# ActiveVisionLab/NeFeS

Measured on AMD Instinct MI355X. Metric: rays/s (fwd+bwd) at 640x480x(64+128) samples, 8x256 MLP, higher is better.
Workload: dtype f32; 1 GPU; BASELINE configs[1]: 7-Scenes-stairs geometry, 64+128 samples, 8x256 MLP + 16-ch feature head; 640x480, random seed-0 weights, fwd + bwd to the 3x4 pose; parallelism=rows/1

## Files before the change

__graft_entry__.py:

```python
import os
import subprocess
import sys

ROOT = os.path.dirname(os.path.abspath(__file__))
if ROOT not in sys.path:
    sys.path.insert(0, ROOT)


def build() -> None:
    env = dict(os.environ)
    env.setdefault("PYTORCH_ROCM_ARCH", "gfx950")
    jobs = str(min(6, os.cpu_count() or 1))
    subprocess.run(["make", "-C", os.path.join(ROOT, "nefes_amd", "csrc"), "-j", jobs], check=True, env=env)
    import py_compile
    for name in ("ref_cpu.py", "refine_cpu.py", "hashgrid_ref.py"):
        py_compile.compile(os.path.join(ROOT, "oracle", name), doraise=True)
    import nefes_amd
    from nefes_amd import lib
    assert lib.load().nefes_version() == lib.ABI_VERSION


def smoke() -> None:
    import torch
    from nefes_amd import lib
    from nefes_amd.field import NeRFH_NFF
    from nefes_amd.render import render
    from oracle import ref_cpu as O
    import types
# ... 43 lines not shown
```

nefes_amd/csrc/field_fwd_h3.hip:

```cpp
#include "field_h3_instances.h"
#ifdef NEFES_TU_W128
#define NEFES_SLAB_KIB 16
#else
#define NEFES_SLAB_KIB 32
#endif
#include <stdio.h>
#include <stdlib.h>
#if defined(NEFES_TU_W128) || !defined(H3_NO_ACC_READ_ASM)
#define NEFES_ASM_READS_ACC
#define NEFES_FENCE_TILES
#endif
#if defined(NEFES_TU_W128)
#define NEFES_ACC_VGPR_FORM
#endif

#ifndef NEFES_FWD_CONSUMER_BIAS
#define NEFES_FWD_CONSUMER_BIAS 1
#endif
#include "field_common.h"
#include "../../include/nefes_hip.h"

#include "field_x6.h"
#include "hashgrid.h"
#if !defined(NEFES_TU_W128) && !defined(H3_NO_ACC_READ_ASM)
#define H3_ACC_READ_ASM
#endif
#include "field_h3.h"
#define NEFES_H3_SLOTS 2

struct FieldFwdH3Args {
    const char* stream;
    const float* bias;
    uint32_t n_slabs, bias_floats, scale_off;
    const float* rays_o;
    const float* rays_d;
    const float* z;
    const float* pts;
    const float* xyz_enc;
    const float* viewdirs;
    float* raw_t;
    uint32_t* masks;
    int N, S, R, C;
    long long M;
    int n_tiles;
    uint32_t s_magic, s_shift;
    float* acts;
    int rows;
    int z_row;
    const float2* hg_table;
    HgGeom hg;
    int gout;
};

template <int NT, int T0, int NX>
__device__ __forceinline__ void train_save_h3(float* tile_base, uint32_t voff, int row0, const f32x16 (&X)[NX], float inv) {
    float* p = tile_base + (size_t)(row0 >> 5) * 4096 + voff;
#pragma unroll
    for (int t = 0; t < NT; ++t)
#pragma unroll
        for (int r = 0; r < 16; ++r) {
#ifndef NEFES_TRAIN_NO_STORES
            __builtin_nontemporal_store(X[T0 + t][r] * inv, &p[t * 4096 + nefes_rho(0, r) * 16]);
#endif
        }
}

template <int MODEF, int ENC, int W = 256, int NTR = 1, bool TRAIN = false, bool FH = false>
__global__ __launch_bounds__(256, W == 128 ? 2 : 1) void field_fwd_h3_kernel(FieldFwdH3Args a) {
    constexpr bool FOLD = MODEF == NEFES_FIELD_FULL_FOLD;
    constexpr int MODE = FOLD ? NEFES_FIELD_FULL : MODEF;
    static_assert(NEFES_SLAB_KIB == (W == 128 ? NEFES_H3_FWD_SLAB_KIB_128 : NEFES_H3_FWD_SLAB_KIB), "ring slab size != the packer's for this width");
    static_assert(!FOLD || (MODE != NEFES_FIELD_SIGMA && !TRAIN), "the fold serves the head products of frozen networks");
    constexpr int NTW = W / 32, NTH = W / 64;
    constexpr int ES = ENC != NEFES_XYZ_FREQ10 ? NEFES_X_STEPS : NEFES_E_STEPS;
    constexpr int MW = 8 * (W / 64) + 4 * (W / 128), WT = (NTW + 1) / 2, WH = (NTH + 1) / 2;
    constexpr int NSEG = MODE == NEFES_FIELD_SIGMA ? NEFES_H3F_SIG + 1
                         : (MODE == NEFES_FIELD_STATIC ? NEFES_H3F_N_STATIC : (FOLD ? NEFES_H3FF_N : NEFES_H3F_N));
    extern __shared__ __attribute__((aligned(16))) char smem[];
    char* ring_base = smem;
    float* bias_lds = (float*)(smem + NEFES_H3_SLOTS * NEFES_SLAB_BYTES);
    float* e_lds = bias_lds + ((a.bias_floats + 63) / 64) * 64 + (threadIdx.x >> 6) * (ES * 64) + (threadIdx.x & 63);
    const int lane = threadIdx.x & 63;
    const int wave = __builtin_amdgcn_readfirstlane(threadIdx.x >> 6);
    const int j = lane & 31, h = lane >> 5;
    for (uint32_t i = threadIdx.x; i < a.bias_floats; i += 256) bias_lds[i] = a.bias[i];
    HgGeom* hg_lds = (HgGeom*)(bias_lds + ((a.bias_floats + 63) / 64) * 64 + 4 * ES * 64);
    if constexpr (ENC == NEFES_XYZ_HASHGRID_FUSED) {
        if (threadIdx.x == 0) *hg_lds = a.hg;
    }
    StagedRing ring;
    ring.init(a.stream, a.n_slabs, ring_base, wave, lane);
    const char* ring_lane = ring_base + lane * 16;
    const char* bias_half = (const char*)bias_lds + 16 * h;
    const int* tab_i = (const int*)(bias_lds + a.scale_off);
    const float* tab_f = bias_lds + a.scale_off;
    auto wexp = [&](int seg) { return tab_i[nefes_h3_tab_exp(nefes_h3f_seg(FOLD, seg))]; };
    auto rowb = [&](int seg) { return tab_f[nefes_h3_tab_bound(nefes_h3f_seg(FOLD, seg))]; };
    auto bmax = [&](int blk) { return tab_f[nefes_h3_tab_bias(NSEG, nefes_h3f_bias(FOLD, blk))]; };
    ring.prime(ring_lane);
    constexpr int B_SIG = 8 * W, B_FINAL = B_SIG + 32, B_DIR = B_FINAL + (FOLD ? 0 : W), B_RGB = B_DIR + W / 2,
                  B_T0 = B_RGB + 32 * NTR, B_T1 = B_T0 + W / 2, B_T2 = B_T1 + W / 2, B_TH = B_T2 + W / 2;
#pragma unroll 1
    for (int tile = blockIdx.x; tile < a.n_tiles; tile += gridDim.x) {
        auto locate = [&](uint32_t& m, uint32_t& ray, uint32_t& smp) {
            const uint32_t m_raw = (uint32_t)tile * 128u + (uint32_t)(wave * 32 + j);
            const bool ok = m_raw < (uint32_t)a.M;
            m = ok ? m_raw : (uint32_t)a.M - 1u;
            ray = a.s_magic ? __umulhi(m, a.s_magic) >> a.s_shift : m;
            smp = m - ray * (uint32_t)a.S;
            return ok;
        };
        uint32_t m, ray, smp;
        locate(m, ray, smp);
        float in_o[3] = {0.f, 0.f, 0.f}, in_d[3] = {0.f, 0.f, 0.f}, in_z = 0.f;
// ... 52 lines not shown
            return a.raw_t + ((size_t)rr * a.R * a.S + ss);
        };
        auto bias_at = [&](int off_floats, int es) { return BiasInitScaled{bias_half + off_floats * 4, pow2i(es)}; };
        constexpr bool CB = !TRAIN && W == 256 && NEFES_FWD_CONSUMER_BIAS;
        float2 nbias;
        f32x16 A[NTW], B[NTW];
        uint32_t bits[WT];
        auto clear_bits = [&]() {
#pragma unroll
            for (int w = 0; w < WT; ++w) bits[w] = 0u;
        };
        constexpr bool CAP = MODE != NEFES_FIELD_SIGMA;
        auto tau_of = [&](float M, int ew) {
            const int t = pick_exp(M);
            return t < 100 - ew ? t : 100 - ew;
        };
        auto sigma_head = [&](const f32x16 (&X)[NTW], int es_x, int tau_x) {
            f32x16 sg[1];
            float mdummy = 0.f;
            const int es = tau_x + wexp(NEFES_H3F_SIG);
            if constexpr (CB) {
                const char* bp8 = bias_half + 7 * W * 4;
                nbias = ReluBiasSplitH<false, NTW, WT>::prime(bp8);
                mma_run_h3<1, W / 16, 0, true>(ring, ring_lane, ReluBiasSplitH<false, NTW, WT>{X, bits, pow2i(tau_x - es_x), mdummy, bp8, pow2i(es_x), nbias},
                                               bias_at(B_SIG, es), sg);
            } else
            mma_run_h3<1, W / 16, 0, true>(ring, ring_lane, ReluSplitH<false, NTW, WT>{X, bits, pow2i(tau_x - es_x), mdummy},
                                           bias_at(B_SIG, es), sg);
            float* col = raw_col();
            if (col && h == 0) {
// ... 20 lines not shown
            if constexpr (CB) {                                                                                                \
                const char* bps = bias_half + ((L1_) - 2) * W * 4;                           \
                nbias = ReluBiasSplitH<CAP, NTW, WT>::prime(bps);                                                              \
                mma_run_h3<NTW, W / 16, 0, true>(ring, ring_lane, ReluBiasSplitH<CAP, NTW, WT>{A, bits, pow2i(tau - es_a), mx, bps, pow2i(es_a), nbias}, \
                                                 ZeroInit{}, B);                                                               \
            } else                                                                                                             \
            mma_run_h3<NTW, W / 16, 0, true>(ring, ring_lane, ReluSplitH<CAP, NTW, WT>{A, bits, pow2i(tau - es_a), mx},        \
                                             bias_at(((L1_) - 1) * W, tau + ew), B);                                           \
            M = rb_ * (pair_max(mx) * pow2i(-es_a)) + bm_;                                                                     \
            es_b = tau + ew;                                                                                                   \
            save_trunk(L1_, B, es_b);                                                                                          \
        }                                                                                                                      \
        put_masks(bits, WT);
        constexpr bool END8 = MODE == NEFES_FIELD_SIGMA || FOLD;
        constexpr int NPAIRS = END8 ? 3 : 4;
#pragma unroll 1
        for (int p = 0; p < NPAIRS; ++p) {
            const int l1 = 2 + 2 * p, l2 = l1 + 1;
            const int seg1 = l1 <= 5 ? l1 - 1 : l1;
            const int seg2 = l2 <= 5 ? l2 - 1 : (l2 <= 8 ? l2 : NEFES_H3F_FINAL);
            NEFES_FWD_EVEN_LAYER(l1, seg1)
            clear_bits();
            {
                const int ew = wexp(seg2);
                const int tau = tau_of(p == 1 ? fmaxf(M, mE) : M, ew);
                if (p == 3) sigma_head(B, es_b, tau_of(M, wexp(NEFES_H3F_SIG)));
                const float rb_ = rowb(seg2), bm_ = bmax(l2 <= 8 ? l2 - 1 : NEFES_H3BB_FINAL);
                const float rbe_ = p == 1 ? rowb(NEFES_H3F_L5E) : 0.f;
                float mx = 0.f;
                if constexpr (CB) {
                    const char* bps = bias_half + (l1 - 1) * W * 4;
                    nbias = ReluBiasSplitH<CAP, NTW, WT>::prime(bps);
                    const ReluBiasSplitH<CAP, NTW, WT> src{B, bits, pow2i(tau - es_b), mx, bps, pow2i(es_b), nbias};
                    mma_run_h3<NTW, W / 16, 0, true>(ring, ring_lane, src, ZeroInit{}, A);
                } else
                mma_run_h3<NTW, W / 16, 0, true>(ring, ring_lane, ReluSplitH<CAP, NTW, WT>{B, bits, pow2i(tau - es_b), mx},
                                                 bias_at(l2 <= 8 ? (l2 - 1) * W : B_FINAL, tau + ew), A);
                if (p == 1) mma_run_h3<NTW, ES / 8, 0, false>(ring, ring_lane, LdsSplitH{e_lds, pow2i(tau)}, ZeroInit{}, A);
                M = rb_ * (pair_max(mx) * pow2i(-es_b)) + (p == 1 ? rbe_ * mE : 0.f) + bm_;
                es_a = tau + ew;
                save_trunk(l2, A, es_a);
            }
            put_masks(bits, WT);
        }
        if constexpr (END8) { NEFES_FWD_EVEN_LAYER(8, NEFES_H3F_L8) }
#undef NEFES_FWD_EVEN_LAYER
        if constexpr (MODE == NEFES_FIELD_SIGMA) sigma_head(B, es_b, tau_of(M, wexp(NEFES_H3F_SIG)));
        if constexpr (MODE != NEFES_FIELD_SIGMA) {
            constexpr bool FULL = MODE == NEFES_FIELD_FULL;
            constexpr int NDT = FULL ? 2 * NTH : NTH;
            float v[3];
            {
                uint32_t mm, rr, ss;
                locate(mm, rr, ss);
#pragma unroll
                for (int c = 0; c < 3; ++c) v[c] = a.viewdirs[(size_t)rr * 3 + c];
            }
            float Dv[16];
            {
                float d14[NEFES_D_STEPS];
                embed_slots<NEFES_N_FREQ_DIR>(d14, v, h);
#pragma unroll
// ... 4 lines not shown
#pragma unroll
                for (int s = 0; s < NEFES_D_STEPS; ++s) __builtin_nontemporal_store(Dv[s], &pd[2 * s * 16]);
            }
            f32x16 dt[NDT];
            uint32_t bits2[WH];
            auto clear2 = [&]() {
#pragma unroll
                for (int w = 0; w < WH; ++w) bits2[w] = 0u;
            };
            struct Bias2 {
                BiasInitScaled a, b;
                __device__ __forceinline__ f32x16 operator()(int t) const { return t < NTH ? a(t) : b(t - NTH); }
            };
            int es_dt;
            if constexpr (FOLD) {
                sigma_head(B, es_b, tau_of(M, wexp(NEFES_H3F_SIG)));
                const int ew = wexp(NEFES_H3F_DT_H);
                const float mD = pair_max(array_max(Dv));
                const int tau = tau_of(fmaxf(M, mD), ew);
                const float rbh_ = rowb(NEFES_H3F_DT_H), rbd_ = rowb(NEFES_H3F_DT_D);
                const float bm_ = fmaxf(bmax(NEFES_H3BB_DIR), bmax(NEFES_H3BB_T0));
                float mx = 0.f;
                es_dt = tau + ew;
                clear_bits();
                if constexpr (CB) {
                    const char* bp8 = bias_half + 7 * W * 4;
                    nbias = ReluBiasSplitH<CAP, NTW, WT>::prime(bp8);
                    const ReluBiasSplitH<CAP, NTW, WT> src8{B, bits, pow2i(tau - es_b), mx, bp8, pow2i(es_b), nbias};
                    mma_run_h3<NDT, W / 16, 0, true>(ring, ring_lane, src8, Bias2{bias_at(B_DIR, es_dt), bias_at(B_T0, es_dt)}, dt);
                } else {
                    const ReluSplitH<CAP, NTW, WT> src8{B, bits, pow2i(tau - es_b), mx};
                    mma_run_h3<NDT, W / 16, 0, true>(ring, ring_lane, src8, Bias2{bias_at(B_DIR, es_dt), bias_at(B_T0, es_dt)}, dt);
                }
                mma_run_h3<NDT, 2, 0, false>(ring, ring_lane, ArraySplitH<16>{Dv, pow2i(tau)}, ZeroInit{}, dt);
                M = rbh_ * (pair_max(mx) * pow2i(-es_b)) + rbd_ * mD + bm_;
                put_masks(bits, WT);
            } else {
                const int ew = wexp(NEFES_H3F_DT_H);
                const float mD = pair_max(array_max(Dv));
                const int tau = tau_of(fmaxf(M, mD), ew);
                float mx = 0.f;
                es_dt = tau + ew;
                if constexpr (CB) {
                    const char* bpf = bias_half + B_FINAL * 4;
                    nbias = ReluBiasSplitH<false, 1, 1>::prime(bpf);
                    const IdentBiasSplitH<NTW> srcf{A, pow2i(tau - es_a), mx, bpf, pow2i(es_a), nbias};
                    if constexpr (FULL) mma_run_h3<NDT, W / 16, 0, true>(ring, ring_lane, srcf, Bias2{bias_at(B_DIR, es_dt), bias_at(B_T0, es_dt)}, dt);
                    else mma_run_h3<NDT, W / 16, 0, true>(ring, ring_lane, srcf, bias_at(B_DIR, es_dt), dt);
// ... 109 lines not shown
    }
}

static void magic_div(uint32_t d, uint32_t& magic, uint32_t& shift) {
    if (d == 1) { magic = 0; shift = 0; return; }
    uint32_t l = 0;
    while ((1ull << l) < d) ++l;
    const uint64_t p = 31 + l;
    magic = (uint32_t)(((1ull << p) + d - 1) / d);
    shift = (uint32_t)(p - 32);
}

template <int MODE, int ENC, int W = 256, int NTR = 1, bool TRAIN = false, bool FH = false>
static int launch_h3(const FieldFwdH3Args& a, hipStream_t st) {
    constexpr int ES_ = ENC != NEFES_XYZ_FREQ10 ? NEFES_X_STEPS : NEFES_E_STEPS;
    const size_t lds = (size_t)NEFES_H3_SLOTS * NEFES_SLAB_BYTES + ((a.bias_floats + 63) / 64) * 256 + (size_t)4 * ES_ * 64 * 4
                       + (ENC == NEFES_XYZ_HASHGRID_FUSED ? 512 : 0);
    static_assert(sizeof(HgGeom) <= 512, "the level geometry's LDS slot");
    auto k = field_fwd_h3_kernel<MODE, ENC, W, NTR, TRAIN, FH>;
    hipError_t e = hipFuncSetAttribute((const void*)k, hipFuncAttributeMaxDynamicSharedMemorySize, (int)lds);
    if (e != hipSuccess) return (int)e;
    int dev = 0, cus = 256;
    (void)hipGetDevice(&dev);
    (void)hipDeviceGetAttribute(&cus, hipDeviceAttributeMultiprocessorCount, dev);
    const int per_cu = W == 128 ? 2 : 1;
    int grid = a.n_tiles < cus * per_cu ? a.n_tiles : cus * per_cu;
    if (const char* cap = getenv("NEFES_DEBUG_MAX_GRID")) {
        const int c = atoi(cap);
        if (c > 0 && c < grid) grid = c;
    }
    hipLaunchKernelGGL(k, dim3(grid), dim3(256), lds, st, a);
// ... 77 lines not shown
    int rc = nefes_blob_info(desc, &info);
    if (rc) return rc;
    *si = info.stream[k.mode == NEFES_FIELD_SIGMA ? NEFES_STREAM_FWD_SIGMA_H3
                      : (k.mode == NEFES_FIELD_STATIC ? NEFES_STREAM_FWD_STATIC_H3 : NEFES_STREAM_FWD_FULL_H3)];
    return si->n_slabs == 0 ? NEFES_E_UNSUPPORTED : 0;
}

static int h3_fwd_args(const NefesNetDesc* desc, const void* packed, const NefesH3FwdKey& k, int N, int S,
                       const NefesHashGridDesc* grid, FieldFwdH3Args& a) {
    NefesStreamInfo si;
    int rc = h3_fwd_stream(desc, k, &si);
    if (rc) return rc;
    a.stream = (const char*)packed + si.slab_off;
    a.bias = (const float*)((const char*)packed + si.bias_off);
    a.n_slabs = si.n_slabs; a.bias_floats = si.bias_floats; a.scale_off = si.scale_off;
    if (k.enc == NEFES_XYZ_HASHGRID_FUSED) {
        rc = hg_geometry(grid, &a.hg, nullptr);
        if (rc) return rc;
        if (a.hg.n_levels != 16) return NEFES_E_UNSUPPORTED;
    }
    a.gout = k.fh ? k.w / 2 : 0;
    a.N = N; a.S = S; a.C = k.fh ? a.gout + 1 : desc->feat_dim;
    a.R = k.mode == NEFES_FIELD_SIGMA ? 1 : 3 + a.C + (k.mode == NEFES_FIELD_STATIC ? 1 : 6);
    a.M = (long long)N * S;
    if (a.M >= (1ll << 31) - 256) return NEFES_E_UNSUPPORTED;
    a.n_tiles = (int)((a.M + 127) / 128);
    a.rows = k.train ? nefes_train_row(desc->width, desc->feat_dim, NEFES_TB_END) : 0;
    magic_div((uint32_t)S, a.s_magic, a.s_shift);
    return 0;
}
// ... 99 lines not shown
```

nefes_amd/csrc/field_h3.h:

```cpp
#pragma once
#ifndef NEFES_H3_WIDE_MIN
#define NEFES_H3_WIDE_MIN 8
#endif
#ifndef NEFES_H3_WIDE_MAX
#define NEFES_H3_WIDE_MAX 64
#endif

typedef _Float16 f16x8 __attribute__((ext_vector_type(8)));

struct Split2 {
    u32x4 h, l;
};
__device__ __forceinline__ f16x8 as_f16x8(u32x4 v) {
    f16x8 r;
    __builtin_memcpy(&r, &v, 16);
    return r;
}
__device__ __forceinline__ f16x8 as_f16x8(f32x4 v) {
    f16x8 r;
    __builtin_memcpy(&r, &v, 16);
    return r;
}

__device__ __forceinline__ float pow2i(int e) {
// ... 81 lines not shown
    o.l[p] = l;
}

struct PairRegs {
    float x0, x1;
};
__device__ __forceinline__ float acc_read(const float& x) {
#if defined(H3_ACC_READ_ASM)
    float v;
    asm volatile("v_accvgpr_read_b32 %0, %1" : "=v"(v) : "a"(x));
    return v;
#else
    return x;
#endif
}
template <bool CAPTURE, int NX, int NWORDS, int T0 = 0>
struct ReluSplitH {
    const f32x16 (&X)[NX];
    uint32_t (&bits)[NWORDS];
    float r;
    float& m;
    __device__ __forceinline__ void stage_a(PairRegs& s, int q, int p) const {
        s.x0 = acc_read(X[T0 + (q >> 1)][(q & 1) * 8 + 2 * p]);
        s.x1 = acc_read(X[T0 + (q >> 1)][(q & 1) * 8 + 2 * p + 1]);
        if (CAPTURE) {
            mask_shift_in(bits[(8 * q + 2 * p) >> 5], s.x0);
            mask_shift_in(bits[(8 * q + 2 * p + 1) >> 5], s.x1);
        }
    }
    __device__ __forceinline__ void stage_b(PairRegs& s) const {
        s.x0 = relu1<false>(s.x0);
        s.x1 = relu1<false>(s.x1);
        max3_acc(m, s.x0, s.x1);
    }
    template <bool NOP>
    __device__ __forceinline__ void stage_c(Split2& o, int p, const PairRegs& s) const { split_pair_h<NOP>(o, p, s.x0, s.x1, r); }
    __device__ __forceinline__ void stage_c1(Split2& o, int p, const PairRegs& s) const { split_pair_hi(o, p, s.x0, s.x1, r); }
    template <bool NOP>
    __device__ __forceinline__ void stage_c2(Split2& o, int p, const PairRegs& s) const { split_pair_lo<NOP>(o, p, s.x0, s.x1, r); }
};
template <bool CAPTURE, int NX, int NWORDS>
struct ReluBiasSplitH {
    const f32x16 (&X)[NX];
    uint32_t (&bits)[NWORDS];
    float r;
    float& m;
    const char* bp;
    float bs;
    float2& nb;
    static __device__ __forceinline__ int pair_off(int q, int p) {
        const int r0 = (q & 1) * 8 + 2 * p;
        return ((q >> 1) * 32 + 8 * (r0 >> 2) + (r0 & 3)) * 4;
    }
    static __device__ __forceinline__ float2 prime(const char* bp_) { return *(const float2*)(bp_ + pair_off(0, 0)); }
    __device__ __forceinline__ void stage_a(PairRegs& s, int q, int p) const {
        const float2 b = nb;
        const int qn = p == 3 ? q + 1 : q, pn = p == 3 ? 0 : p + 1;
        nb = *(const float2*)(bp + pair_off(qn, pn));
        s.x0 = __builtin_fmaf(b.x, bs, acc_read(X[q >> 1][(q & 1) * 8 + 2 * p]));
        s.x1 = __builtin_fmaf(b.y, bs, acc_read(X[q >> 1][(q & 1) * 8 + 2 * p + 1]));
        if (CAPTURE) {
            mask_shift_in(bits[(8 * q + 2 * p) >> 5], s.x0);
            mask_shift_in(bits[(8 * q + 2 * p + 1) >> 5], s.x1);
        }
    }
    __device__ __forceinline__ void stage_b(PairRegs& s) const {
        s.x0 = relu1<false>(s.x0);
        s.x1 = relu1<false>(s.x1);
// ... 112 lines not shown

struct BiasInitScaled {
    const char* p;
    float s;
    __device__ __forceinline__ f32x16 operator()(int t) const {
        f32x16 c;
#pragma unroll
        for (int q = 0; q < 4; ++q) {
            const f32x4 b = *(const f32x4*)(p + (t * 32 + 8 * q) * 4);
            c[4 * q + 0] = b[0] * s; c[4 * q + 1] = b[1] * s; c[4 * q + 2] = b[2] * s; c[4 * q + 3] = b[3] * s;
        }
        return c;
    }
};

struct StagedRing {
    const char* src;
    uint32_t n_slabs;
    uint32_t g_next;
    uint32_t c_slot;
    uint32_t cur_off;
    uint32_t my_off;
    char* my_lds;
    f32x4 pf;
    f32x4 stage[NEFES_SLAB_PIECES];

    __device__ __forceinline__ void load_piece(int q) {
        stage[q] = *(const f32x4*)(src + (size_t)g_next * NEFES_SLAB_BYTES + my_off + q * 1024);
    }
    __device__ __forceinline__ void init(const char* stream, uint32_t nslabs, char* ring_base, int wave, int lane) {
        src = stream; n_slabs = nslabs;
        my_off = (uint32_t)(wave * NEFES_SLAB_PIECES * 1024 + lane * 16);
        my_lds = ring_base + my_off;
        g_next = 0; c_slot = 0; cur_off = 0;
#pragma unroll
        for (int q = 0; q < NEFES_SLAB_PIECES; ++q) load_piece(q);
#pragma unroll
        for (int q = 0; q < NEFES_SLAB_PIECES; ++q) *(f32x4*)(my_lds + q * 1024) = stage[q];
        g_next = n_slabs > 1 ? 1 : 0;
#pragma unroll
        for (int q = 0; q < NEFES_SLAB_PIECES; ++q) load_piece(q);
        g_next = (g_next + 1 == n_slabs) ? 0 : g_next + 1;
    }
    __device__ __forceinline__ void store_piece(int q) {
        *(f32x4*)(my_lds + (c_slot ^ 1u) * NEFES_SLAB_BYTES + q * 1024) = stage[q];
    }
    __device__ __forceinline__ void fetch_piece(int q) {
        load_piece(q);
        if (q == NEFES_SLAB_PIECES - 1) g_next = (g_next + 1 == n_slabs) ? 0 : g_next + 1;
    }
    __device__ __forceinline__ void issue_piece(int q) {
        *(f32x4*)(my_lds + (c_slot ^ 1u) * NEFES_SLAB_BYTES + q * 1024) = stage[q];
        load_piece(q);
        if (q == NEFES_SLAB_PIECES - 1) g_next = (g_next + 1 == n_slabs) ? 0 : g_next + 1;
    }
    __device__ __forceinline__ uint32_t acquire() {
        asm volatile("s_waitcnt lgkmcnt(0)" ::: "memory");
        __builtin_amdgcn_s_barrier();
        c_slot ^= 1u;
        return c_slot * NEFES_SLAB_BYTES;
    }
    __device__ __forceinline__ void prime(const char* ring_lane) {
        asm volatile("s_waitcnt lgkmcnt(0)" ::: "memory");
        __builtin_amdgcn_s_barrier();
        cur_off = 0;
        pf = *(const f32x4*)(ring_lane);
    }
    __device__ __forceinline__ void drain() {}
};

__device__ __forceinline__ void mfma_h3_asm(f32x16& c, const f32x4& a, const u32x4& b) {
    asm volatile("v_mfma_f32_32x32x16_f16 %0, %1, %2, %0" : "+a"(c) : "v"(a), "v"(b));
}
__device__ __forceinline__ void mfma_h3_asm_v(f32x16& c, const f32x4& a, const u32x4& b) {
    asm volatile("v_mfma_f32_32x32x16_f16 %0, %1, %2, %0" : "+v"(c) : "v"(a), "v"(b));
}
__device__ __forceinline__ void mfma_h3_asm_c0(f32x16& c, const f32x4& a, const u32x4& b) {
    asm volatile("v_mfma_f32_32x32x16_f16 %0, %1, %2, 0" : "=a"(c) : "v"(a), "v"(b));
}
__device__ __forceinline__ void mfma_h3_asm_v_c0(f32x16& c, const f32x4& a, const u32x4& b) {
    asm volatile("v_mfma_f32_32x32x16_f16 %0, %1, %2, 0" : "=v"(c) : "v"(a), "v"(b));
}
template <class T> struct h3_is_zero_init { static constexpr bool value = false; };
template <> struct h3_is_zero_init<ZeroInit> { static constexpr bool value = true; };
// ... 8 lines not shown
    constexpr int NSLAB = (NU + UPS - 1) / UPS;
    Split2 B0, B1;
    auto BQ = [&](int k) -> Split2& { return (k & 1) ? B1 : B0; };
    asm volatile("s_nop 13" ::: "memory");
#ifdef H3_WIDE_ENTRY_FENCE
    __builtin_amdgcn_sched_barrier(0);
    asm volatile("s_nop 7\n\ts_nop 7\n\ts_nop 1" ::: "memory");
    __builtin_amdgcn_sched_barrier(0);
#endif
    {
        PairRegs s0;
#pragma unroll
        for (int pp = 0; pp < 4; ++pp) {
            src.stage_a(s0, 0, pp);
            src.stage_b(s0);
            if (pp == 3) src.template stage_c<true>(B0, pp, s0);
            else src.template stage_c<false>(B0, pp, s0);
        }
    }
    constexpr bool C0 = FIRST && h3_is_zero_init<InitFn>::value
        ;
    if (FIRST && !C0) acc[T0] = init(0);
    const char* p = ring_lane + ring.cur_off;
    f32x4 ha0 = ring.pf, la0 = *(const f32x4*)(p + 1024);
    f32x4 ha1 = *(const f32x4*)(p + 2048), la1 = *(const f32x4*)(p + 3072);
    f32x4 ha2, la2;
    auto HA = [&](int k) -> f32x4& { return k % 3 == 0 ? ha0 : (k % 3 == 1 ? ha1 : ha2); };
    auto LA = [&](int k) -> f32x4& { return k % 3 == 0 ? la0 : (k % 3 == 1 ? la1 : la2); };
    PairRegs ps[4];
#pragma unroll
// ... 25 lines not shown
                    }
                    if (vt) mfma_h3_asm_v(acc[T0 + t], l0, B.h);
                    else mfma_h3_asm(acc[T0 + t], l0, B.h);
                }
                __builtin_amdgcn_sched_barrier(0);
                if (host) src.stage_a(ps[pp], q + 1, pp);
                if (tail) src.template stage_c2<false>(Bn, pp, ps[pp]);
                if (!host && uu != acq_u) h2 = *(const f32x4*)(pn);
                __builtin_amdgcn_sched_barrier(0);
                asm volatile("" ::"v"(l0), "v"(B.h));
                if (vt) mfma_h3_asm_v(acc[T0 + t], h0, B.l);
                else mfma_h3_asm(acc[T0 + t], h0, B.l);
                __builtin_amdgcn_sched_barrier(0);
                if (host) src.stage_b(ps[pp]);
                if (host && uu != acq_u) h2 = *(const f32x4*)(pn);
                if (!host) {
#pragma unroll
                    for (int qq = 0; qq < NEFES_SLAB_PIECES; ++qq)
                        if (piece_unit(qq) == uu) ring.store_piece(qq);
                }
                if (FIRST && !C0 && q == 0 && t + 1 < NT) {
                    acc[T0 + t + 1] = init(t + 1);
                }
                __builtin_amdgcn_sched_barrier(0);
                asm volatile("" ::"v"(B.l));
                if (vt) mfma_h3_asm_v(acc[T0 + t], h0, B.h);
                else mfma_h3_asm(acc[T0 + t], h0, B.h);
                __builtin_amdgcn_sched_barrier(0);
                if (host) src.stage_c1(Bn, pp, ps[pp]);
                if (!host) {
// ... 28 lines not shown

template <int NT, int KS16, int T0, bool FIRST = true, class SrcFn, class InitFn, int NACC, class Ring>
__device__ __forceinline__ void mma_run_h3_small(Ring& ring, const char* ring_lane, const SrcFn& src, const InitFn& init,
                                           f32x16 (&acc)[NACC]) {
    static_assert(T0 + NT <= NACC, "accumulator array too small");
    constexpr int UPS = (NEFES_SLAB_FRAGS / 4) / 2;
    constexpr int NU = KS16 * NT;
    constexpr int NSLAB = (NU + UPS - 1) / UPS;
    Split2 B, Bn;
    {
        PairRegs s0;
#pragma unroll
        for (int pp = 0; pp < 4; ++pp) {
            src.stage_a(s0, 0, pp);
            src.stage_b(s0);
            if (pp == 3) src.template stage_c<true>(B, pp, s0);
            else src.template stage_c<false>(B, pp, s0);
        }
    }
    Bn = B;
    if (FIRST) acc[T0] = init(0);
    const char* p = ring_lane + ring.cur_off;
    f32x4 ah = ring.pf, al = *(const f32x4*)(p + 1024);
#pragma unroll
    for (int sl = 0; sl < NSLAB; ++sl) {
        const int nu = (NU - sl * UPS) < UPS ? (NU - sl * UPS) : UPS;
#pragma unroll
        for (int uu = 0; uu < UPS; ++uu) {
            if (uu < nu) {
                const int u = sl * UPS + uu, q = u / NT, t = u % NT;
// ... 25 lines not shown
                            ring.issue_piece(qq);
                            __builtin_amdgcn_sched_barrier(0);
                        }
                }
                c = __builtin_amdgcn_mfma_f32_32x32x16_f16(Ah, Bl, c, 0, 0, 0);
                c = __builtin_amdgcn_mfma_f32_32x32x16_f16(Ah, Bh, c, 0, 0, 0);
                acc[T0 + t] = c;
                if (q + 1 < KS16) {
                    constexpr int STRIDE = NT >= 8 ? 2 : 1;
#pragma unroll
                    for (int pp = 0; pp < 4; ++pp)
                        if (NT >= 4 ? (t == pp * STRIDE + STRIDE - 1) : (t == (pp * NT) / 4)) {
                            PairRegs s1;
                            src.stage_a(s1, q + 1, pp);
                            src.stage_b(s1);
                            if (pp == 3) src.template stage_c<true>(Bn, pp, s1);
                            else src.template stage_c<false>(Bn, pp, s1);
#pragma unroll
                            for (int i = 0; i < 2; ++i) {
                                __builtin_amdgcn_sched_group_barrier(0x008, 1, 0);
                                __builtin_amdgcn_sched_group_barrier(0x002, 4, 0);
                            }
                        }
                }
                ah = nh;
            }
        }
    }
    ring.pf = ah;
    mfma_results_fence_tiles<12, NT, T0>(acc);
// ... 9 lines not shown
```

Measured before the change: 738,700 rays/s.

## Compute sigma head as an FP32 dot product fused into the next layer's staging

Instead of running the sigma head as a separate MFMA pass over a streamed weight slab, the forward kernel preloads the sigma weights into LDS as FP32. It accumulates the dot product with the ReLU'd trunk activations while they are staged for the following layer's matmul, finishing with a cross-half permlane swap. The weight ring now skips the sigma slab. This removes one slab fetch and a small MFMA run per tile, at the cost of extra FMAs and LDS reads inside the staging loop, more register pressure, and a slightly different rounding path.

```diff
diff --git a/__graft_entry__.py b/__graft_entry__.py
--- a/__graft_entry__.py
+++ b/__graft_entry__.py
@@ -11,7 +11,7 @@
     env = dict(os.environ)
     env.setdefault("PYTORCH_ROCM_ARCH", "gfx950")
     jobs = str(min(6, os.cpu_count() or 1))
-    subprocess.run(["make", "-C", os.path.join(ROOT, "nefes_amd", "csrc"), "-j", jobs], check=True, env=env)
+    subprocess.run(["make", "-C", os.path.join(ROOT, "nefes_amd", "csrc"), "-j", jobs, "all", "nodot"], check=True, env=env)
     import py_compile
     for name in ("ref_cpu.py", "refine_cpu.py", "hashgrid_ref.py"):
         py_compile.compile(os.path.join(ROOT, "oracle", name), doraise=True)
diff --git a/nefes_amd/csrc/field_fwd_h3.hip b/nefes_amd/csrc/field_fwd_h3.hip
--- a/nefes_amd/csrc/field_fwd_h3.hip
+++ b/nefes_amd/csrc/field_fwd_h3.hip
@@ -17,6 +17,9 @@
 #ifndef NEFES_FWD_CONSUMER_BIAS
 #define NEFES_FWD_CONSUMER_BIAS 1
 #endif
+#ifndef NEFES_FWD_SIGMA_DOT
+#define NEFES_FWD_SIGMA_DOT 1
+#endif
 #include "field_common.h"
 #include "../../include/nefes_hip.h"
 
@@ -27,6 +30,8 @@
 #endif
 #include "field_h3.h"
 #define NEFES_H3_SLOTS 2
+
+constexpr bool h3_fwd_sigma_dot(bool train) { return NEFES_FWD_SIGMA_DOT && !train; }
 
 struct FieldFwdH3Args {
     const char* stream;
@@ -50,6 +55,7 @@
     const float2* hg_table;
     HgGeom hg;
     int gout;
+    uint32_t sig_slab;
 };
 
 template <int NT, int T0, int NX>
@@ -71,6 +77,10 @@
     constexpr int MODE = FOLD ? NEFES_FIELD_FULL : MODEF;
     static_assert(NEFES_SLAB_KIB == (W == 128 ? NEFES_H3_FWD_SLAB_KIB_128 : NEFES_H3_FWD_SLAB_KIB), "ring slab size != the packer's for this width");
     static_assert(!FOLD || (MODE != NEFES_FIELD_SIGMA && !TRAIN), "the fold serves the head products of frozen networks");
+    constexpr bool DOT = h3_fwd_sigma_dot(TRAIN);
+    static_assert(!DOT || (W / 16) * 2048 == NEFES_SLAB_BYTES, "static_sigma's segment is not one slab of this stream");
+    static_assert(!DOT || !TRAIN, "TRAIN instances keep static_sigma's own run");
+    constexpr int WSIG_BYTES = DOT ? W * 4 : 0;
     constexpr int NTW = W / 32, NTH = W / 64;
     constexpr int ES = ENC != NEFES_XYZ_FREQ10 ? NEFES_X_STEPS : NEFES_E_STEPS;
     constexpr int MW = 8 * (W / 64) + 4 * (W / 128), WT = (NTW + 1) / 2, WH = (NTH + 1) / 2;
@@ -78,7 +88,8 @@
                          : (MODE == NEFES_FIELD_STATIC ? NEFES_H3F_N_STATIC : (FOLD ? NEFES_H3FF_N : NEFES_H3F_N));
     extern __shared__ __attribute__((aligned(16))) char smem[];
     char* ring_base = smem;
-    float* bias_lds = (float*)(smem + NEFES_H3_SLOTS * NEFES_SLAB_BYTES);
+    float* wsig_lds = (float*)(smem + NEFES_H3_SLOTS * NEFES_SLAB_BYTES);
+    float* bias_lds = (float*)(smem + NEFES_H3_SLOTS * NEFES_SLAB_BYTES + WSIG_BYTES);
     float* e_lds = bias_lds + ((a.bias_floats + 63) / 64) * 64 + (threadIdx.x >> 6) * (ES * 64) + (threadIdx.x & 63);
     const int lane = threadIdx.x & 63;
     const int wave = __builtin_amdgcn_readfirstlane(threadIdx.x >> 6);
@@ -88,16 +99,27 @@
     if constexpr (ENC == NEFES_XYZ_HASHGRID_FUSED) {
         if (threadIdx.x == 0) *hg_lds = a.hg;
     }
-    StagedRing ring;
-    ring.init(a.stream, a.n_slabs, ring_base, wave, lane);
+    StagedRingT<DOT> ring;
+    ring.init(a.stream, a.n_slabs, ring_base, wave, lane, a.sig_slab);
     const char* ring_lane = ring_base + lane * 16;
-    const char* bias_half = (const char*)bias_lds + 16 * h;
+    const char* wsig_half = (const char*)wsig_lds + 16 * h;
+    const char* bias_half = wsig_half + WSIG_BYTES;
     const int* tab_i = (const int*)(bias_lds + a.scale_off);
     const float* tab_f = bias_lds + a.scale_off;
     auto wexp = [&](int seg) { return tab_i[nefes_h3_tab_exp(nefes_h3f_seg(FOLD, seg))]; };
     auto rowb = [&](int seg) { return tab_f[nefes_h3_tab_bound(nefes_h3f_seg(FOLD, seg))]; };
     auto bmax = [&](int blk) { return tab_f[nefes_h3_tab_bias(NSEG, nefes_h3f_bias(FOLD, blk))]; };
     ring.prime(ring_lane);
+    if constexpr (DOT) {
+        const float sc = pow2i(-wexp(NEFES_H3F_SIG));
+        const char* seg = a.stream + (size_t)a.sig_slab * NEFES_SLAB_BYTES;
+        for (int c = threadIdx.x; c < W; c += 256) {
+            const int wi = c & 31, s = 16 * (c >> 5) + nefes_row_reg(wi);
+            const _Float16* u = (const _Float16*)(seg + (s >> 3) * 2048) + 256 * nefes_row_half(wi) + (s & 7);
+            wsig_lds[c] = ((float)u[0] + (float)u[512]) * sc;
+        }
+        __syncthreads();
+    }
     constexpr int B_SIG = 8 * W, B_FINAL = B_SIG + 32, B_DIR = B_FINAL + (FOLD ? 0 : W), B_RGB = B_DIR + W / 2,
                   B_T0 = B_RGB + 32 * NTR, B_T1 = B_T0 + W / 2, B_T2 = B_T1 + W / 2, B_TH = B_T2 + W / 2;
 #pragma unroll 1
@@ -180,6 +202,42 @@
         auto tau_of = [&](float M, int ew) {
             const int t = pick_exp(M);
             return t < 100 - ew ? t : 100 - ew;
+        };
+        auto sigma_close = [&](float t, int es_x) {
+            const uint32_t u = __float_as_uint(t);
+            const auto r = __builtin_amdgcn_permlane32_swap(u, u, false, false);
+            const float pre = (__uint_as_float(r[0]) + __uint_as_float(r[1])) * pow2i(-es_x) + bias_lds[B_SIG];
+            float* col = raw_col();
+            if (col && h == 0) {
+                const int ch = (MODE == NEFES_FIELD_SIGMA) ? 0 : 3 + a.C;
+                __builtin_nontemporal_store(softplus_ref(pre), &col[(size_t)ch * a.S]);
+            }
+        };
+        auto sigma_dot_loop = [&](const f32x16 (&X)[NTW], int es_x) {
+            float s0 = 0.f, s1 = 0.f, tot = 0.f;
+            const float bs = pow2i(es_x);
+            __builtin_amdgcn_sched_barrier(0);
+#pragma unroll
+            for (int t = 0; t < NTW; ++t) {
+#pragma unroll
+                for (int g = 0; g < 8; ++g) {
+                    const int off = (t * 32 + 8 * (g >> 1) + 2 * (g & 1)) * 4;
+                    const float2 w = *(const float2*)(wsig_half + off);
+                    float x0 = acc_read(X[t][2 * g]), x1 = acc_read(X[t][2 * g + 1]);
+                    if constexpr (CB) {
+                        const float2 b = *(const float2*)(bias_half + 7 * W * 4 + off);
+                        x0 = __builtin_fmaf(b.x, bs, x0);
+                        x1 = __builtin_fmaf(b.y, bs, x1);
+                    }
+                    x0 = relu1<false>(x0);
+                    x1 = relu1<false>(x1);
+                    s0 = g == 0 ? x0 * w.x : __builtin_fmaf(x0, w.x, s0);
+                    s1 = g == 0 ? x1 * w.y : __builtin_fmaf(x1, w.y, s1);
+                }
+                tot = tot + (s0 + s1);
+            }
+            __builtin_amdgcn_sched_barrier(0);
+            sigma_close(tot, es_x);
         };
         auto sigma_head = [&](const f32x16 (&X)[NTW], int es_x, int tau_x) {
             f32x16 sg[1];
@@ -230,38 +288,59 @@
         put_masks(bits, WT);
         constexpr bool END8 = MODE == NEFES_FIELD_SIGMA || FOLD;
         constexpr int NPAIRS = END8 ? 3 : 4;
+        constexpr bool PEEL = DOT && !END8 && W == 128;
+#define NEFES_FWD_ODD_LAYER(p, l1, l2, seg2, D_)                                                                               \
+        clear_bits();                                                                                                          \
+        {                                                                                                                      \
+            const int ew = wexp(seg2);                                                                                         \
+             \
+            const int tau = tau_of((p) == 1 ? fmaxf(M, mE) : M, ew);                                                           \
+            if (!(D_) && !PEEL && (p) == 3) {                                              \
+                if constexpr (DOT) sigma_dot_loop(B, es_b);                                                                    \
+                else sigma_head(B, es_b, tau_of(M, wexp(NEFES_H3F_SIG)));                                                      \
+            }                                                                                                                  \
+            const float rb_ = rowb(seg2), bm_ = bmax((l2) <= 8 ? (l2) - 1 : NEFES_H3BB_FINAL);       \
+            const float rbe_ = (p) == 1 ? rowb(NEFES_H3F_L5E) : 0.f;                                                           \
+            float mx = 0.f, sg0 = 0.f, sg1 = 0.f, sgt = 0.f;                                                                            \
+            float2 nwsig = {0.f, 0.f};                                                                                         \
+            if constexpr (D_) nwsig = *(const float2*)(wsig_half + h3_pair_off(0, 0));                                         \
+            if constexpr (CB) {                                                                                                \
+                const char* bps = bias_half + ((l1) - 1) * W * 4;                          \
+                nbias = ReluBiasSplitH<CAP, NTW, WT>::prime(bps);                                                              \
+                const ReluBiasSplitH<CAP, NTW, WT, D_> src{B, bits, pow2i(tau - es_b), mx, bps, pow2i(es_b), nbias,            \
+                                                           sigma_dot_refs<D_>(wsig_half, nwsig, sg0, sg1, sgt)};                    \
+                mma_run_h3<NTW, W / 16, 0, true>(ring, ring_lane, src, ZeroInit{}, A);        \
+            } else {                                                                                                           \
+                const ReluSplitH<CAP, NTW, WT, 0, D_> src{B, bits, pow2i(tau - es_b), mx, sigma_dot_refs<D_>(wsig_half, nwsig, sg0, sg1, sgt)}; \
+                mma_run_h3<NTW, W / 16, 0, true>(ring, ring_lane, src,                                                         \
+                                                 bias_at((l2) <= 8 ? ((l2) - 1) * W : B_FINAL, tau + ew), A);    \
+            }                                                                                                                  \
+            if constexpr (D_) sigma_close(sgt, es_b);                                                                           \
+            if ((p) == 1) mma_run_h3<NTW, ES / 8, 0, false>(ring, ring_lane, LdsSplitH{e_lds, pow2i(tau)}, ZeroInit{}, A);    \
+            M = rb_ * (pair_max(mx) * pow2i(-es_b)) + ((p) == 1 ? rbe_ * mE : 0.f) + bm_;                                      \
+            es_a = tau + ew;                                                                                                   \
+            save_trunk(l2, A, es_a);                                                                                           \
+        }                                                                                                                      \
+        put_masks(bits, WT);
 #pragma unroll 1
-        for (int p = 0; p < NPAIRS; ++p) {
+        for (int p = 0; p < (PEEL ? 3 : NPAIRS); ++p) {
             const int l1 = 2 + 2 * p, l2 = l1 + 1;
             const int seg1 = l1 <= 5 ? l1 - 1 : l1;
             const int seg2 = l2 <= 5 ? l2 - 1 : (l2 <= 8 ? l2 : NEFES_H3F_FINAL);
             NEFES_FWD_EVEN_LAYER(l1, seg1)
-            clear_bits();
-            {
-                const int ew = wexp(seg2);
-                const int tau = tau_of(p == 1 ? fmaxf(M, mE) : M, ew);
-                if (p == 3) sigma_head(B, es_b, tau_of(M, wexp(NEFES_H3F_SIG)));
-                const float rb_ = rowb(seg2), bm_ = bmax(l2 <= 8 ? l2 - 1 : NEFES_H3BB_FINAL);
-                const float rbe_ = p == 1 ? rowb(NEFES_H3F_L5E) : 0.f;
-                float mx = 0.f;
-                if constexpr (CB) {
-                    const char* bps = bias_half + (l1 - 1) * W * 4;
-                    nbias = ReluBiasSplitH<CAP, NTW, WT>::prime(bps);
-                    const ReluBiasSplitH<CAP, NTW, WT> src{B, bits, pow2i(tau - es_b), mx, bps, pow2i(es_b), nbias};
-                    mma_run_h3<NTW, W / 16, 0, true>(ring, ring_lane, src, ZeroInit{}, A);
-                } else
-                mma_run_h3<NTW, W / 16, 0, true>(ring, ring_lane, ReluSplitH<CAP, NTW, WT>{B, bits, pow2i(tau - es_b), mx},
-                                                 bias_at(l2 <= 8 ? (l2 - 1) * W : B_FINAL, tau + ew), A);
-                if (p == 1) mma_run_h3<NTW, ES / 8, 0, false>(ring, ring_lane, LdsSplitH{e_lds, pow2i(tau)}, ZeroInit{}, A);
-                M = rb_ * (pair_max(mx) * pow2i(-es_b)) + (p == 1 ? rbe_ * mE : 0.f) + bm_;
-                es_a = tau + ew;
-                save_trunk(l2, A, es_a);
-            }
-            put_masks(bits, WT);
-        }
+            NEFES_FWD_ODD_LAYER(p, l1, l2, seg2, false)
+        }
+        if constexpr (PEEL) {
+            NEFES_FWD_EVEN_LAYER(8, NEFES_H3F_L8)
+            NEFES_FWD_ODD_LAYER(3, 8, 9, NEFES_H3F_FINAL, true)
+        }
+#undef NEFES_FWD_ODD_LAYER
         if constexpr (END8) { NEFES_FWD_EVEN_LAYER(8, NEFES_H3F_L8) }
 #undef NEFES_FWD_EVEN_LAYER
-        if constexpr (MODE == NEFES_FIELD_SIGMA) sigma_head(B, es_b, tau_of(M, wexp(NEFES_H3F_SIG)));
+        if constexpr (MODE == NEFES_FIELD_SIGMA) {
+            if constexpr (DOT) sigma_dot_loop(B, es_b);
+            else sigma_head(B, es_b, tau_of(M, wexp(NEFES_H3F_SIG)));
+        }
         if constexpr (MODE != NEFES_FIELD_SIGMA) {
             constexpr bool FULL = MODE == NEFES_FIELD_FULL;
             constexpr int NDT = FULL ? 2 * NTH : NTH;
@@ -296,7 +375,10 @@
             };
             int es_dt;
             if constexpr (FOLD) {
-                sigma_head(B, es_b, tau_of(M, wexp(NEFES_H3F_SIG)));
+                if constexpr (!DOT) sigma_head(B, es_b, tau_of(M, wexp(NEFES_H3F_SIG)));
+                float sg0 = 0.f, sg1 = 0.f, sgt = 0.f;
+                float2 nwsig = {0.f, 0.f};
+                if constexpr (DOT) nwsig = *(const float2*)(wsig_half + h3_pair_off(0, 0));
                 const int ew = wexp(NEFES_H3F_DT_H);
                 const float mD = pair_max(array_max(Dv));
                 const int tau = tau_of(fmaxf(M, mD), ew);
@@ -308,12 +390,14 @@
                 if constexpr (CB) {
                     const char* bp8 = bias_half + 7 * W * 4;
                     nbias = ReluBiasSplitH<CAP, NTW, WT>::prime(bp8);
-                    const ReluBiasSplitH<CAP, NTW, WT> src8{B, bits, pow2i(tau - es_b), mx, bp8, pow2i(es_b), nbias};
+                    const ReluBiasSplitH<CAP, NTW, WT, DOT> src8{B, bits, pow2i(tau - es_b), mx, bp8, pow2i(es_b), nbias,
+                                                                 sigma_dot_refs<DOT>(wsig_half, nwsig, sg0, sg1, sgt)};
                     mma_run_h3<NDT, W / 16, 0, true>(ring, ring_lane, src8, Bias2{bias_at(B_DIR, es_dt), bias_at(B_T0, es_dt)}, dt);
                 } else {
-                    const ReluSplitH<CAP, NTW, WT> src8{B, bits, pow2i(tau - es_b), mx};
+                    const ReluSplitH<CAP, NTW, WT, 0, DOT> src8{B, bits, pow2i(tau - es_b), mx, sigma_dot_refs<DOT>(wsig_half, nwsig, sg0, sg1, sgt)};
                     mma_run_h3<NDT, W / 16, 0, true>(ring, ring_lane, src8, Bias2{bias_at(B_DIR, es_dt), bias_at(B_T0, es_dt)}, dt);
                 }
+                if constexpr (DOT) sigma_close(sgt, es_b);
                 mma_run_h3<NDT, 2, 0, false>(ring, ring_lane, ArraySplitH<16>{Dv, pow2i(tau)}, ZeroInit{}, dt);
                 M = rbh_ * (pair_max(mx) * pow2i(-es_b)) + rbd_ * mD + bm_;
                 put_masks(bits, WT);
@@ -453,7 +537,8 @@
 template <int MODE, int ENC, int W = 256, int NTR = 1, bool TRAIN = false, bool FH = false>
 static int launch_h3(const FieldFwdH3Args& a, hipStream_t st) {
     constexpr int ES_ = ENC != NEFES_XYZ_FREQ10 ? NEFES_X_STEPS : NEFES_E_STEPS;
-    const size_t lds = (size_t)NEFES_H3_SLOTS * NEFES_SLAB_BYTES + ((a.bias_floats + 63) / 64) * 256 + (size_t)4 * ES_ * 64 * 4
+    const size_t lds = (size_t)NEFES_H3_SLOTS * NEFES_SLAB_BYTES + (h3_fwd_sigma_dot(TRAIN) ? W * 4 : 0)
+                       + ((a.bias_floats + 63) / 64) * 256 + (size_t)4 * ES_ * 64 * 4
                        + (ENC == NEFES_XYZ_HASHGRID_FUSED ? 512 : 0);
     static_assert(sizeof(HgGeom) <= 512, "the level geometry's LDS slot");
     auto k = field_fwd_h3_kernel<MODE, ENC, W, NTR, TRAIN, FH>;
@@ -561,6 +646,15 @@
     a.stream = (const char*)packed + si.slab_off;
     a.bias = (const float*)((const char*)packed + si.bias_off);
     a.n_slabs = si.n_slabs; a.bias_floats = si.bias_floats; a.scale_off = si.scale_off;
+    a.sig_slab = ~0u;
+    if (h3_fwd_sigma_dot(k.train != 0)) {
+        NefesBlobInfo info;
+        rc = nefes_blob_info(desc, &info);
+        if (rc) return rc;
+        const uint32_t n_sig = info.stream[NEFES_STREAM_FWD_SIGMA_H3].n_slabs;
+        if (n_sig < 3 || n_sig > si.n_slabs) return NEFES_E_UNSUPPORTED;
+        a.sig_slab = n_sig - 1;
+    }
     if (k.enc == NEFES_XYZ_HASHGRID_FUSED) {
         rc = hg_geometry(grid, &a.hg, nullptr);
         if (rc) return rc;
diff --git a/nefes_amd/csrc/field_h3.h b/nefes_amd/csrc/field_h3.h
--- a/nefes_amd/csrc/field_h3.h
+++ b/nefes_amd/csrc/field_h3.h
@@ -119,12 +119,57 @@
     return x;
 #endif
 }
-template <bool CAPTURE, int NX, int NWORDS, int T0 = 0>
+template <bool DOT>
+struct SigmaDotRefs {};
+template <>
+struct SigmaDotRefs<true> {
+    const char* wp;
+    float2& nw;
+    float& s0;
+    float& s1;
+    float& t;
+};
+__device__ __forceinline__ int h3_pair_off(int q, int p) {
+    const int r0 = (q & 1) * 8 + 2 * p;
+    return ((q >> 1) * 32 + 8 * (r0 >> 2) + (r0 & 3)) * 4;
+}
+template <bool DOT>
+__device__ __forceinline__ void sigma_dot_pair(const SigmaDotRefs<DOT>& d, const PairRegs& s, int q, int p) {
+    if constexpr (DOT) {
+        const float2 w = d.nw;
+        const int qn = p == 3 ? q + 1 : q, pn = p == 3 ? 0 : p + 1;
+        d.nw = *(const float2*)(d.wp + h3_pair_off(qn, pn));
+        if ((q & 1) == 0 && p == 0) {
+            d.s0 = s.x0 * w.x;
+            d.s1 = s.x1 * w.y;
+        } else {
+            d.s0 = __builtin_fmaf(s.x0, w.x, d.s0);
+            d.s1 = __builtin_fmaf(s.x1, w.y, d.s1);
+        }
+        if ((q & 1) == 1 && p == 3) d.t = d.t + (d.s0 + d.s1);
+    }
+}
+template <bool DOT>
+__device__ __forceinline__ SigmaDotRefs<DOT> sigma_dot_refs(const char* wp, float2& nw, float& s0, float& s1, float& t) {
+    if constexpr (DOT) return {wp, nw, s0, s1, t};
+    else return {};
+}
+template <class T, class = void>
+struct h3_src_dot { static constexpr bool value = false; };
+template <class T>
+struct h3_src_dot<T, decltype((void)T::kDot)> { static constexpr bool value = T::kDot; };
+template <class SrcFn>
+__device__ __forceinline__ void h3_stage_d(const SrcFn& src, const PairRegs& s, int q, int p) {
+    if constexpr (h3_src_dot<SrcFn>::value) sigma_dot_pair(src.dot, s, q, p);
+}
+template <bool CAPTURE, int NX, int NWORDS, int T0 = 0, bool DOT = false>
 struct ReluSplitH {
+    static constexpr bool kDot = DOT;
     const f32x16 (&X)[NX];
     uint32_t (&bits)[NWORDS];
     float r;
     float& m;
+    SigmaDotRefs<DOT> dot;
     __device__ __forceinline__ void stage_a(PairRegs& s, int q, int p) const {
         s.x0 = acc_read(X[T0 + (q >> 1)][(q & 1) * 8 + 2 * p]);
         s.x1 = acc_read(X[T0 + (q >> 1)][(q & 1) * 8 + 2 * p + 1]);
@@ -144,8 +189,9 @@
     template <bool NOP>
     __device__ __forceinline__ void stage_c2(Split2& o, int p, const PairRegs& s) const { split_pair_lo<NOP>(o, p, s.x0, s.x1, r); }
 };
-template <bool CAPTURE, int NX, int NWORDS>
+template <bool CAPTURE, int NX, int NWORDS, bool DOT = false>
 struct ReluBiasSplitH {
+    static constexpr bool kDot = DOT;
     const f32x16 (&X)[NX];
     uint32_t (&bits)[NWORDS];
     float r;
@@ -153,10 +199,8 @@
     const char* bp;
     float bs;
     float2& nb;
-    static __device__ __forceinline__ int pair_off(int q, int p) {
-        const int r0 = (q & 1) * 8 + 2 * p;
-        return ((q >> 1) * 32 + 8 * (r0 >> 2) + (r0 & 3)) * 4;
-    }
+    SigmaDotRefs<DOT> dot;
+    static __device__ __forceinline__ int pair_off(int q, int p) { return h3_pair_off(q, p); }
     static __device__ __forceinline__ float2 prime(const char* bp_) { return *(const float2*)(bp_ + pair_off(0, 0)); }
     __device__ __forceinline__ void stage_a(PairRegs& s, int q, int p) const {
         const float2 b = nb;
@@ -299,7 +343,8 @@
     }
 };
 
-struct StagedRing {
+template <bool SKIP = false>
+struct StagedRingT {
     const char* src;
     uint32_t n_slabs;
     uint32_t g_next;
@@ -309,12 +354,18 @@
     char* my_lds;
     f32x4 pf;
     f32x4 stage[NEFES_SLAB_PIECES];
+    uint32_t skip;
 
     __device__ __forceinline__ void load_piece(int q) {
         stage[q] = *(const f32x4*)(src + (size_t)g_next * NEFES_SLAB_BYTES + my_off + q * 1024);
     }
-    __device__ __forceinline__ void init(const char* stream, uint32_t nslabs, char* ring_base, int wave, int lane) {
-        src = stream; n_slabs = nslabs;
+    __device__ __forceinline__ void advance() {
+        uint32_t g = g_next + 1;
+        if (SKIP && g == skip) ++g;
+        g_next = g >= n_slabs ? 0 : g;
+    }
+    __device__ __forceinline__ void init(const char* stream, uint32_t nslabs, char* ring_base, int wave, int lane, uint32_t skip_slab = ~0u) {
+        src = stream; n_slabs = nslabs; skip = skip_slab;
         my_off = (uint32_t)(wave * NEFES_SLAB_PIECES * 1024 + lane * 16);
         my_lds = ring_base + my_off;
         g_next = 0; c_slot = 0; cur_off = 0;
@@ -322,22 +373,22 @@
         for (int q = 0; q < NEFES_SLAB_PIECES; ++q) load_piece(q);
 #pragma unroll
         for (int q = 0; q < NEFES_SLAB_PIECES; ++q) *(f32x4*)(my_lds + q * 1024) = stage[q];
-        g_next = n_slabs > 1 ? 1 : 0;
+        if (SKIP) advance(); else g_next = n_slabs > 1 ? 1 : 0;
 #pragma unroll
         for (int q = 0; q < NEFES_SLAB_PIECES; ++q) load_piece(q);
-        g_next = (g_next + 1 == n_slabs) ? 0 : g_next + 1;
+        if (SKIP) advance(); else g_next = (g_next + 1 == n_slabs) ? 0 : g_next + 1;
     }
     __device__ __forceinline__ void store_piece(int q) {
         *(f32x4*)(my_lds + (c_slot ^ 1u) * NEFES_SLAB_BYTES + q * 1024) = stage[q];
     }
     __device__ __forceinline__ void fetch_piece(int q) {
         load_piece(q);
-        if (q == NEFES_SLAB_PIECES - 1) g_next = (g_next + 1 == n_slabs) ? 0 : g_next + 1;
+        if (q == NEFES_SLAB_PIECES - 1) { if (SKIP) advance(); else g_next = (g_next + 1 == n_slabs) ? 0 : g_next + 1; }
     }
     __device__ __forceinline__ void issue_piece(int q) {
         *(f32x4*)(my_lds + (c_slot ^ 1u) * NEFES_SLAB_BYTES + q * 1024) = stage[q];
         load_piece(q);
-        if (q == NEFES_SLAB_PIECES - 1) g_next = (g_next + 1 == n_slabs) ? 0 : g_next + 1;
+        if (q == NEFES_SLAB_PIECES - 1) { if (SKIP) advance(); else g_next = (g_next + 1 == n_slabs) ? 0 : g_next + 1; }
     }
     __device__ __forceinline__ uint32_t acquire() {
         asm volatile("s_waitcnt lgkmcnt(0)" ::: "memory");
@@ -353,6 +404,7 @@
     }
     __device__ __forceinline__ void drain() {}
 };
+using StagedRing = StagedRingT<false>;
 
 __device__ __forceinline__ void mfma_h3_asm(f32x16& c, const f32x4& a, const u32x4& b) {
     asm volatile("v_mfma_f32_32x32x16_f16 %0, %1, %2, %0" : "+a"(c) : "v"(a), "v"(b));
@@ -391,6 +443,7 @@
         for (int pp = 0; pp < 4; ++pp) {
             src.stage_a(s0, 0, pp);
             src.stage_b(s0);
+            h3_stage_d(src, s0, 0, pp);
             if (pp == 3) src.template stage_c<true>(B0, pp, s0);
             else src.template stage_c<false>(B0, pp, s0);
         }
@@ -446,6 +499,7 @@
                 __builtin_amdgcn_sched_barrier(0);
                 if (host) src.stage_b(ps[pp]);
                 if (host && uu != acq_u) h2 = *(const f32x4*)(pn);
+                if (tail) h3_stage_d(src, ps[pp], q + 1, pp);
                 if (!host) {
 #pragma unroll
                     for (int qq = 0; qq < NEFES_SLAB_PIECES; ++qq)
@@ -504,6 +558,7 @@
         for (int pp = 0; pp < 4; ++pp) {
             src.stage_a(s0, 0, pp);
             src.stage_b(s0);
+            h3_stage_d(src, s0, 0, pp);
             if (pp == 3) src.template stage_c<true>(B, pp, s0);
             else src.template stage_c<false>(B, pp, s0);
         }
@@ -559,6 +614,7 @@
                             PairRegs s1;
                             src.stage_a(s1, q + 1, pp);
                             src.stage_b(s1);
+                            h3_stage_d(src, s1, q + 1, pp);
                             if (pp == 3) src.template stage_c<true>(Bn, pp, s1);
                             else src.template stage_c<false>(Bn, pp, s1);
 #pragma unroll
```

Result: no change. 745,000 rays/s (median of 6 runs) (+0.8%).
